# willake/cpu-ray-tracer

Measured on AMD Instinct MI355X. Metric: Mrays/sec (primary+secondary), 1280x720 64spp path trace — pipelined throughput over 878 consecutive 64-spp windows of one progressive render (single_render = one such render alone), higher is better.
Workload: dtype f32; 1 GPU; bunny_scene.xml FileScene BVH-SAH path tracer, 1280x720, 64 spp/step (passes=1, depthLimit=5); 1 step = 64 frames = the next spp window of a progressive render; the 878 steps are one crt_render job (14 render kernel launch(es), a wavefront per (tile, 128 consecutive frames), + ordered accumulate), one sync at the end; triangles=4968, parallelism=tile-wave x1

## Files before the change

cpu-ray-tracer_amd/__init__.py:

```python
import ctypes as C
import os
import subprocess

import numpy as np

HERE = os.path.dirname(os.path.abspath(__file__))
REPO = os.path.dirname(HERE)
LIB_PATH = os.environ.get("CRT_LIB_PATH") or os.path.join(HERE, "libcrt_amd.so")

SCENE_FILE, SCENE_TLAS = 0, 1
UPDATE_TRANSFORMS, UPDATE_BOUNDS = 1, 2
ACCEL_KDTREE, ACCEL_GRID = 1, 2
KD_NODE_DTYPE = np.dtype([("aabbMin", "<f4", 3), ("left", "<i4"), ("aabbMax", "<f4", 3), ("right", "<i4"), ("splitDistance", "<f4"), ("splitAxis", "<i4"),
                          ("firstTri", "<u4"), ("triCount", "<u4")])


class CrtError(RuntimeError):
    def __init__(self, code, msg):
        super().__init__("crt error %d: %s" % (code, msg))
        self.code = code


class Config(C.Structure):
    _fields_ = [("width", C.c_int32), ("height", C.c_int32), ("depthLimit", C.c_int32), ("device", C.c_int32),
# ... 516 lines not shown
        side = getattr(self, "_side_stream", None)
        if side is None:
            side = self._side_stream = torch.cuda.Stream(device=self.device)
        side.wait_stream(st)
        with torch.cuda.stream(side):
            out = run(side)
        st.wait_stream(side)
        for t in (out if isinstance(out, tuple) else (out,)):
            if isinstance(t, torch.Tensor):
                t.record_stream(st)
        return out

    def counters(self):
        c = CountersS()
        self._ck(self.L.crt_get_counters(self.h, C.byref(c)))
        return {n: int(getattr(c, n)) for n, _ in c._fields_}

    def reset_counters(self):
        self._ck(self.L.crt_reset_counters(self.h))

    def timing(self):
        t = TimingS()
        self._ck(self.L.crt_get_timing(self.h, C.byref(t)))
        return dict(render_kernel_ms=t.render_kernel_ms, resolve_kernel_ms=t.resolve_kernel_ms, render_launches=t.render_launches, pool_launches=t.pool_launches, split_launches=t.split_launches)

    def pool_lds(self, frames):
        self.L.crt_debug_pool_lds.restype = C.c_int
        self.L.crt_debug_pool_lds.argtypes = [C.c_void_p, C.c_uint32, C.c_void_p, C.c_void_p, C.c_void_p]
        b, lim, bits = C.c_uint32(), C.c_uint32(), C.c_uint32()
        if self.L.crt_debug_pool_lds(self.h, int(frames), C.byref(b), C.byref(lim), C.byref(bits)) != 0:
            raise CrtError(-3, "pool_lds: no scene uploaded")
        return b.value, lim.value, bits.value

    def tile_classes(self):
        self.L.crt_debug_tile_classes.restype = C.c_int
        self.L.crt_debug_tile_classes.argtypes = [C.c_void_p, C.c_void_p, C.c_uint32]
        n = self.L.crt_debug_tile_classes(self.h, None, 0)
        if n < 0:
            self._ck(n)
        out = np.zeros(n, np.uint8)
        if n:
            rc = self.L.crt_debug_tile_classes(self.h, _p(out), n)
            if rc < 0:
                self._ck(rc)
        return out

    def tile_clocks(self, tile_count):
        a = np.zeros((tile_count, 2), np.uint64)
        self._ck(self.L.crt_get_tile_clocks(self.h, _p(a)))
        return a

    def bind_accumulator(self, device_ptr):
        self._ck(self.L.crt_bind_accumulator(self.h, C.c_void_p(device_ptr)))

    def accumulator_device_ptr(self):
        p = C.c_void_p()
        self._ck(self.L.crt_accumulator_device_ptr(self.h, C.byref(p)))
        return p.value

def hit_fields(hits):
    import torch
    i = hits.view(torch.int32)
    return dict(t=hits[:, 0], u=hits[:, 1], v=hits[:, 2], objIdx=i[:, 3], triIdx=i[:, 4], traversed=i[:, 5], tested=i[:, 6])


def hit_info_fields(info):
    import torch
    return dict(I=info[:, 0:3], material=info.view(torch.int32)[:, 3], N=info[:, 4:7], u=info[:, 7], albedo=info[:, 8:11], v=info[:, 11])


class HostScene:

    def __init__(self, xml_path, kind, base_dir=None):
        self.L = lib()
        h = C.c_void_p()
# ... 325 lines not shown
def host_kd_build(positions):
    pos = np.ascontiguousarray(positions, np.float32).reshape(-1, 9)
    L = lib()
    info = (C.c_uint32 * 4)()

    def ck(rc):
        if rc != 0:
            raise CrtError(rc, L.crt_host_last_error().decode())
    ck(L.crt_host_kd_build(_p(pos), C.c_uint32(len(pos)), info, None, None))
    nodes = np.zeros(info[0], KD_NODE_DTYPE); r = np.zeros(max(info[1], 1), np.uint32)
    ck(L.crt_host_kd_build(_p(pos), C.c_uint32(len(pos)), None, _p(nodes), _p(r)))
    return dict(nodes=nodes, refs=r[:info[1]], maxDepth=int(info[2]), nodesUsed=int(info[3]))


def host_vertex_dedup(v8):
    v8 = np.ascontiguousarray(v8, np.float32).reshape(-1, 8)
    idx = np.zeros(len(v8), np.uint32); uniq = np.zeros((len(v8), 8), np.float32)
    L = lib(); L.crt_host_vertex_dedup.restype = C.c_uint32
    n = L.crt_host_vertex_dedup(v8.ctypes.data_as(C.c_void_p), C.c_uint32(len(v8)), idx.ctypes.data_as(C.c_void_p), uniq.ctypes.data_as(C.c_void_p))
    return idx, uniq[:n].copy()


def spp_window(rank, frames_per_rank, first_spp=1):
    return first_spp + rank * frames_per_rank


def tile_partition(rank, world, n_tiles):
    count = (n_tiles - rank + world - 1) // world if rank < n_tiles else 0
    return rank, world, count


TILE_NO_LIGHT, TILE_NO_FLOOR, TILE_NO_TREE = 1, 2, 4
TILE_SKY = 7


def tile_classes_host(camera, light_offsets, light_size, floor_d, root_pair, width, height, tile_first=0, tile_stride=1, tile_count=-1, flags=7):
    if tile_count < 0:
        tile_first, tile_stride, tile_count = 0, 1, (width // 16) * (height // 16)
    v = np.concatenate([np.asarray(camera, np.float32).reshape(12), np.asarray(light_offsets, np.float32).reshape(3), np.array([light_size, floor_d], np.float32),
                        np.asarray(root_pair, np.float32).reshape(16)]).astype(np.float32)
    out = np.zeros(tile_count, np.uint8)
    L = lib()
    L.crt_debug_tile_classes_host.restype = C.c_int
    L.crt_debug_tile_classes_host.argtypes = [C.c_void_p, C.c_uint32, C.c_int, C.c_int, C.c_uint32, C.c_uint32, C.c_uint32, C.c_void_p]
    rc = L.crt_debug_tile_classes_host(_p(v), flags, width, height, tile_first, tile_stride, tile_count, _p(out))
    if rc != 0:
        raise CrtError(rc, "crt_debug_tile_classes_host: invalid argument")
    return out


def reduce_accumulator(tensor, dist, dst=0):
    dist.reduce(tensor, dst=dst, op=dist.ReduceOp.SUM)
    return tensor


def allreduce_accumulator(tensor, dist):
    dist.all_reduce(tensor, op=dist.ReduceOp.SUM)
    return tensor
```

cpu-ray-tracer_amd/csrc/abi.cpp:

```cpp
#include "../../include/crt_abi.h"
#include "device/launch.h"
#include "device/tile_class.h"
#include "device/build_common.h"
#include "host/grid_resolution.h"

#include <cmath>
#include <cstdarg>
#include <cstddef>
#include <cstdio>
#include <cstdlib>
#include <cstring>
#include <deque>
#include <string>
#include <algorithm>
#include <vector>
#include <chrono>

static_assert(sizeof(crt_bvh_node) == 32 && sizeof(crt_tri) == 112 && sizeof(crt_tlas_node) == 32, "reference layouts");
static_assert(sizeof(crt::NodePair) == 64 && sizeof(crt::LeafTri) == 48 && sizeof(crt::ShadeTri) == 64 && sizeof(crt::TlasNode) == 32 &&
              sizeof(crt::Instance) == 128 && sizeof(crt::Material) == 32 && offsetof(crt::Instance, T) == 64, "device layouts");
static_assert(sizeof(crt_counters) == sizeof(crt::Counters), "counter layout");
static_assert(sizeof(crt_kd_node) == 48 && sizeof(crt::KdNode) == sizeof(crt_kd_node) && sizeof(crt::AltTri) == 48, "flat KD node (uploaded as it comes), alternative accelerators' triangle record");
static_assert(offsetof(crt::PrimDev, red) == 536 && sizeof(crt::PrimDev) == 552, "PrimDev: 134 floats, then the two texel pointers");
static_assert(sizeof(crt::BlasAltDesc) == 72, "BLAS descriptor");
// ... 957 lines not shown
    };
    float world[24];
    for (int i = 0; i < 8; i++) { world[3 * i] = (i & 1) ? c->meshHi[0] : c->meshLo[0]; world[3 * i + 1] = (i & 2) ? c->meshHi[1] : c->meshLo[1]; world[3 * i + 2] = (i & 4) ? c->meshHi[2] : c->meshLo[2]; }
    int wr[4] = {0, c->tilesX - 1, 0, c->tilesY - 1};
    (void)rect_of(world, wr);
    std::vector<uint32_t> first, second, rest;
    for (uint32_t i = 0; i < c->tileCount; i++) {
        const uint32_t tile = c->tileFirst + i * c->tileStride;
        const int tx = (int)(tile % (uint32_t)c->tilesX), ty = (int)(tile / (uint32_t)c->tilesX);
        const bool inRect = tx >= wr[0] && tx <= wr[1] && ty >= wr[2] && ty <= wr[3];
        if (inRect) first.push_back(i); else rest.push_back(i);
    }
    for (int k = 0; k <= crt_ctx::kLatStages; k++) { c->tuneCount[k] = 0; c->tuneMs[k] = 0; }
    c->latStage = 0; c->latBest = 0; c->latDone = false; c->latWarm = false; c->latConfirming = false; c->latQueue.clear(); c->costPending = false; c->latProbed = false;
    first.insert(first.end(), rest.begin(), rest.end());
    (void)sky_to_tail(c->hostClass, first);
    c->jobCostValid = false; c->jobCostPending = false; c->planValid = false; c->skyWindowTicks = 0;
    { const int r = upload_tile_order(c, first); if (r) return r; }
    c->orderDirty = false;
    return 0;
}

static int update_tile_class(crt_ctx* c)
{
    if (!c->classDirty || c->tileCount == 0) return 0;
    if (!c->dTileClass) HIPCK(c, hipMalloc((void**)&c->dTileClass, (size_t)c->tileCount));
    { const int r = order_behind_ahead(c); if (r) return r; }
    const int k = c->classFlip ^= 1;
    if (!c->hTileClass[k]) {
        HIPCK(c, hipHostMalloc((void**)&c->hTileClass[k], (size_t)c->tileCount, hipHostMallocDefault));
        HIPCK(c, ensure_event(&c->classCopied[k]));
    } else HIPCK(c, hipEventSynchronize(c->classCopied[k]));
    crt::classify_tiles(c->hScene, c->cfg.width, c->cfg.height, (uint32_t)c->tilesX, c->tileFirst, c->tileStride, c->tileCount, c->hTileClass[k]);
    {
        const uint8_t* cls = c->hTileClass[k];
        bool same = c->hostClass.size() == c->tileCount; uint32_t sky = 0;
        for (uint32_t i = 0; i < c->tileCount; i++) { const bool s = cls[i] == crt::kTileSky; sky += s ? 1u : 0u; if (same && s != (c->hostClass[i] == crt::kTileSky)) same = false; }
        c->hostClass.assign(cls, cls + c->tileCount); c->skyTiles = sky;
        if (!same) c->orderDirty = true;
    }
    HIPCK(c, hipMemcpyAsync(c->dTileClass, c->hTileClass[k], (size_t)c->tileCount, hipMemcpyHostToDevice, c->stream));
    HIPCK(c, hipEventRecord(c->classCopied[k], c->stream));
    c->orderReady = c->classCopied[k];
    c->classDirty = false;
    return 0;
}

static size_t sample_bytes_per_window(const crt_ctx* c, uint32_t passes) { return crt_slab_window_bytes(c->tileCount, passes); }
static size_t window_bytes(const crt_ctx* c, uint32_t passes) { return sample_bytes_per_window(c, passes) + (c->usePool ? crt_pool_scratch_bytes_per_window(c->tileCount) : 0); }

static uint32_t block_desc(uint32_t tile, uint32_t laneBase, uint32_t lanes, uint32_t window) { uint32_t lg = 0; while ((1u << lg) < lanes) lg++; return tile | (laneBase << 16) | (lg << 22) | (window << 25); }
static const uint32_t kLatLanes[7] = {64u, 32u, 16u, 8u, 4u, 2u, 1u};
static const double kLatG[7] = {1.0, 0.93, 0.88, 0.79, 0.69, 0.57, 0.48};
static int lat_index(uint32_t L) { int k = 0; while (k < 6 && kLatLanes[k] != L) k++; return k; }

static uint8_t next_lanes(uint8_t lanes, uint32_t cost, double T)
{
    int k = lat_index(lanes); const double unit = (double)cost / kLatG[k];
    while (k < 6 && unit * kLatG[k] > T) k++;
    while (k > 0 && unit * kLatG[k - 1] <= 0.9 * T) k--;
    return (uint8_t)kLatLanes[k];
}
extern "C" int crt_debug_next_lanes(const uint8_t* lanes, const uint32_t* cost, uint32_t n, double T, uint8_t* out)
{
    if (!lanes || !cost || !out) return CRT_ERR_INVALID;
    for (uint32_t i = 0; i < n; i++) { if (lanes[i] == 0 || lanes[i] > 64 || (64 % lanes[i]) != 0) return CRT_ERR_INVALID; out[i] = next_lanes(lanes[i], cost[i], T); }
// ... 2232 lines not shown
    if (e == hipSuccess) e = crt_launch_check_sqrt(d, c->stream);
    if (e == hipSuccess) e = hipMemcpyAsync(out, d, 16, hipMemcpyDeviceToHost, c->stream);
    if (e == hipSuccess) e = hipStreamSynchronize(c->stream);
    (void)hipFree(d);
    HIPCK(c, e);
    return CRT_OK;
}

extern "C" int crt_debug_primary_block(crt_ctx* c, float* out, float* camera, float* lightFloor)
{
    if (!c || !out) return CRT_ERR_INVALID;
    const crt::Scene& s = c->hScene;
    static_assert(offsetof(crt::Scene, primRoot) == offsetof(crt::Scene, rootPair) + 64 && offsetof(crt::Scene, primDown) + 12 == offsetof(crt::Scene, rootPair) + 64 + 4 * crt::kPrimFloats, "primary block");
    memcpy(out, s.rootPair, 64 + 4 * crt::kPrimFloats);
    if (camera) memcpy(camera, s.camPos, 48);
    if (lightFloor) { lightFloor[0] = s.lightInvT[7]; lightFloor[1] = s.lightInvT[3]; lightFloor[2] = s.lightInvT[11]; lightFloor[3] = s.floorD; }
    return CRT_OK;
}
extern "C" int crt_debug_primary_block_host(int op, const float* in, float* out)
{
    static crt::Scene s{};
    if (!in || !out || op < 0 || op > 2) return CRT_ERR_INVALID;
    if (op == 0) {
        s = crt::Scene{};
        s.camPos[2] = -2; s.topLeft[0] = -1; s.topLeft[1] = 1; s.topRight[0] = 1; s.topRight[1] = 1; s.bottomLeft[0] = -1; s.bottomLeft[1] = -1;
        memcpy(s.lightInvT, in, 48); s.floorD = in[12]; memcpy(s.rootPair, in + 13, 64); s.rootIsPair = 1;
    } else if (op == 1) { memcpy(s.camPos, in, 12); memcpy(s.topLeft, in + 3, 12); memcpy(s.topRight, in + 6, 12); memcpy(s.bottomLeft, in + 9, 12); }
    else memcpy(s.rootPair, in, 64);
    crt::set_primary(s);
    memcpy(out, s.rootPair, 64 + 4 * crt::kPrimFloats);
    return CRT_OK;
}

extern "C" int crt_debug_tile_classes(crt_ctx* c, uint8_t* out, uint32_t cap)
{
    if (!c || (!out && cap)) return CRT_ERR_INVALID;
    HIPCK(c, hipSetDevice(c->cfg.device));
    { const int r = update_tile_class(c); if (r) return r; }
    const uint32_t n = cap < c->tileCount ? cap : c->tileCount;
    if (n) {
        HIPCK(c, hipMemcpyAsync(out, c->dTileClass, n, hipMemcpyDeviceToHost, c->stream));
        HIPCK(c, hipStreamSynchronize(c->stream));
    }
    return (int)c->tileCount;
}
extern "C" int crt_debug_tile_classes_host(const float* in, uint32_t flags, int W, int H, uint32_t tileFirst, uint32_t tileStride, uint32_t tileCount, uint8_t* out)
{
    if (!in || !out || W < 16 || H < 16 || tileStride == 0) return CRT_ERR_INVALID;
    const uint32_t tilesX = (uint32_t)(W / 16), tiles = tilesX * (uint32_t)(H / 16);
    if (tileCount && (unsigned long long)tileFirst + (unsigned long long)(tileCount - 1) * tileStride >= tiles) return CRT_ERR_INVALID;
    crt::Scene s{};
    memcpy(s.camPos, in, 12); memcpy(s.topLeft, in + 3, 12); memcpy(s.topRight, in + 6, 12); memcpy(s.bottomLeft, in + 9, 12);
    s.W = W; s.H = H; s.invW = 1.0f / W; s.invH = 1.0f / H;
    s.lightInvT[0] = s.lightInvT[5] = s.lightInvT[10] = 1.0f; s.lightInvT[3] = in[12]; s.lightInvT[7] = in[13]; s.lightInvT[11] = in[14];
    s.lightSize = in[15]; s.floorN[1] = 1.0f; s.floorD = in[16];
    memcpy(s.rootPair, in + 17, 64);
    s.lightAxis = flags & 1u; s.floorAxisY = (flags >> 1) & 1u; s.rootIsPair = (flags >> 2) & 1u;
    crt::set_primary(s);
    crt::classify_tiles(s, W, H, tilesX, tileFirst, tileStride, tileCount, out);
    return CRT_OK;
}

static int device_probe(crt_ctx* c, int op, const void* in, void* out, uint32_t n)
{
    static const uint8_t words[18][2] = {{1, 1}, {1, 1}, {2, 1}, {1, 1}, {2, 1}, {6, 7}, {1, 18}, {4, 1}, {5, 3}, {13, 2}, {16, 4}, {2, 2}, {2, 2}, {2, 2}, {2, 2}, {4, 2}, {2, 1}, {5, 3}};
    if (!c || !in || !out || op < 0 || op > 17 || n > (1u << 25)) return CRT_ERR_INVALID;
    if (n == 0) return CRT_OK;
    const size_t inBytes = (size_t)n * words[op][0] * 4, outBytes = (size_t)n * words[op][1] * 4;
    HIPCK(c, hipSetDevice(c->cfg.device));
    char* d = nullptr;
    HIPCK(c, hipMalloc((void**)&d, inBytes + outBytes));
    hipError_t e = hipMemcpyAsync(d, in, inBytes, hipMemcpyHostToDevice, c->stream);
    if (e == hipSuccess) e = (op <= 10 || op == 17) ? crt_launch_probe_f32(op, d, d + inBytes, n, c->stream) : crt_launch_probe_f64(op, d, d + inBytes, n, c->stream);
    if (e == hipSuccess) e = hipMemcpyAsync(out, d + inBytes, outBytes, hipMemcpyDeviceToHost, c->stream);
    if (e == hipSuccess) e = hipStreamSynchronize(c->stream);
    (void)hipFree(d);
    HIPCK(c, e);
    return CRT_OK;
}
// ... 126 lines not shown
```

cpu-ray-tracer_amd/csrc/device/layout.h:

```cpp
#pragma once
#include <stdint.h>

namespace crt {

constexpr uint32_t kRefInterior = 0x80000000u;
constexpr uint32_t kRefTlasBit = 0x40000000u;
constexpr uint32_t kRefTlasInterior = 0x40000000u;
constexpr uint32_t kRefTlasLeaf = 0xC0000000u;
constexpr uint32_t kRefReturn = 0xFFFFFFFFu;
constexpr uint32_t kRefDone = 0u;
constexpr uint32_t kRefOffsetMask = 0x3fffffffu;
constexpr uint64_t kMaxGeomBytes = 1ull << 32;

constexpr uint32_t kRef16Interior = 0x8000u, kRef16TlasBit = 0x4000u, kRef16TlasLeaf = 0xC000u, kRef16TagMask = 0xC000u, kRef16IndexMask = 0x3fffu;
constexpr uint32_t kRef16Return = 0xFFFFu, kRef16MaxIndex = 0x3ffeu;
constexpr uint32_t kRefWideMaxIndex = 0x3ffffffeu;
struct PoolRefForm { uint32_t interior, tlasBit, tlasLeaf, tagMask, indexMask, ret; };
constexpr PoolRefForm pool_ref_form(uint32_t bits)
{
    return bits == 32u ? PoolRefForm{kRefInterior, kRefTlasBit, kRefTlasLeaf, 0xC0000000u, kRefOffsetMask, kRefReturn}
                       : PoolRefForm{kRef16Interior, kRef16TlasBit, kRef16TlasLeaf, kRef16TagMask, kRef16IndexMask, kRef16Return};
}

struct alignas(16) NodeChild { float lo[3]; uint32_t ref; float hi[3]; uint32_t ref16; };
// ... 46 lines not shown
    uint32_t tlasOff, instOff, shadeOff;
    uint32_t leafOff, tlasPairOff;
    uint32_t rootRef16, poolRefBits;
    const uint32_t* texels;
    const Material* mats;
    uint32_t rootRef;
    uint32_t stackDepth;
    uint32_t bvhStack;
    uint32_t lightAxis, floorAxisY;
    uint32_t rootIsPair;
    float rootPair[16];
    float primRoot[12];
    float primLight[3];
    float primFloor;
    float primRight[3], primDown[3];
};
constexpr uint32_t kPrimFloats = 22u;

inline void set_primary(Scene& s)
{
    const float* O = s.camPos;
    for (int c = 0; c < 2; c++)
        for (int k = 0; k < 3; k++) {
            s.primRoot[6 * c + k] = s.rootPair[8 * c + k] - O[k];
            s.primRoot[6 * c + 3 + k] = s.rootPair[8 * c + 4 + k] - O[k];
        }
    s.primLight[0] = O[1] + s.lightInvT[7]; s.primLight[1] = O[0] + s.lightInvT[3]; s.primLight[2] = O[2] + s.lightInvT[11];
    s.primFloor = O[1] + s.floorD;
    for (int k = 0; k < 3; k++) { s.primRight[k] = s.topRight[k] - s.topLeft[k]; s.primDown[k] = s.bottomLeft[k] - s.topLeft[k]; }
}

constexpr uint32_t kTileNoLight = 1u, kTileNoFloor = 2u, kTileNoTree = 4u;
constexpr uint32_t kTileSky = kTileNoLight | kTileNoFloor | kTileNoTree;

struct Counters { unsigned long long v[8]; };

struct alignas(16) RefitPlanRec { uint32_t pair, child[2], pad; };
constexpr uint32_t kPlanInterior = 0x80000000u;

struct alignas(64) TlasBuildHeader {
    uint32_t status;
    uint32_t step;
    uint32_t height;
    uint32_t searches;
    uint32_t staleA;
    uint32_t pad[11];
};
constexpr uint32_t kTlasBuildOk = 0u, kTlasBuildNoCandidate = 1u, kTlasBuildNoEnd = 2u;
constexpr uint32_t kTlasMaxBlas = 256u;

#if defined(__HIPCC__)
#define CRT_HOST_DEVICE __host__ __device__
#else
#define CRT_HOST_DEVICE
#endif
template <class TriCountOf>
CRT_HOST_DEVICE inline bool hit_record_ok(int32_t objIdx, int32_t triIdx, uint32_t objects, TriCountOf&& triCountOf)
{
    if (objIdx < 2) return objIdx >= -1;
    if ((uint32_t)(objIdx - 2) >= objects) return false;
    return triIdx >= 0 && (uint32_t)triIdx < triCountOf((uint32_t)(objIdx - 2));
}

struct KdNode { float lo[3]; int32_t left; float hi[3]; int32_t right; float splitDistance; int32_t splitAxis; uint32_t firstTri, triCount; };
struct AltTri { float v0[3]; uint32_t triIdx; float e1[3]; int32_t objIdx; float e2[3]; uint32_t pad; };
struct AltAccelDev {
// ... 57 lines not shown
```

cpu-ray-tracer_amd/csrc/device/render_pool.hip:

```cpp
#include <type_traits>
#include "launch.h"
#include "sample_body.h"

namespace crt {

enum : uint32_t {
    F_OX = 0, F_OY, F_OZ, F_DX, F_DY, F_DZ,
    F_RX, F_RY, F_RZ,
    F_T,
    F_SEED, F_META,
    F_U, F_V,
    F_COUNT,
    F_CUR = F_U, F_PEND = F_V,
    F_TRI = F_RX
};
constexpr uint32_t kMetaItemMask = 0x7ffu, kMetaDepthShift = 11u, kMetaInside = 1u << 14, kMetaFresh = 1u << 15, kMetaObjShift = 16u, kMetaLowMask = 0xffffu;
constexpr uint32_t kQueueMask = 127u;

#ifndef CRT_POOL_MIN_WAVES
#define CRT_POOL_MIN_WAVES 4
#endif
#ifndef CRT_POOL_WIDE_MIN_WAVES
#define CRT_POOL_WIDE_MIN_WAVES 4
#endif
// ... 45 lines not shown
__device__ __forceinline__ uint32_t rank_in(uint64_t m) { return __builtin_amdgcn_mbcnt_hi((uint32_t)(m >> 32), __builtin_amdgcn_mbcnt_lo((uint32_t)m, 0u)); }

template <int KIND, bool COUNT, int S, int REFBITS = 16>
__global__ __launch_bounds__(64, REFBITS == 32 ? CRT_POOL_WIDE_MIN_WAVES : CRT_POOL_MIN_WAVES) void render_pool_kernel(const Scene sc, char* __restrict__ slab, float* __restrict__ facScratch, Counters* __restrict__ counters,
                                                             unsigned long long* __restrict__ tileClocks, const uint32_t* __restrict__ tileOrder,
                                                             uint32_t tileFirst, uint32_t tileStride, uint32_t tileCount, uint32_t tilesX,
                                                             uint32_t sppFirst, uint32_t frames, uint32_t passes, uint32_t groups, uint32_t waveFrames, const uint32_t* __restrict__ waveTab, uint32_t tabBlocks, uint32_t longFrames,
                                                             uint32_t rankFirst, uint32_t* __restrict__ tileCost, unsigned long long* __restrict__ launchClk, const uint8_t* __restrict__ tileClass)
{
    extern __shared__ uint32_t lds[];
    const uint32_t lane = threadIdx.x;
#ifdef CRT_POOL_TIMELINE
    const unsigned long long tl0 = wall_clock64();
#endif
    const unsigned long long clk0 = (COUNT || tileCost) ? wall_clock64() : 0ull;
    if (launchClk && lane == 0) { atomicMax(&launchClk[0], ~clk0); atomicMax(&launchClk[1], clk0); }
    uint32_t rank0, grp, wf = waveFrames, first = 0u, limit = frames;
    if (waveTab) {
        if (blockIdx.x < tabBlocks) {
            uint32_t lo = 0u, hi = tileCount - rankFirst;
            while (hi - lo > 1u) { const uint32_t mid = (lo + hi) >> 1; if (waveTab[2u * mid] <= blockIdx.x) lo = mid; else hi = mid; }
            rank0 = lo; grp = blockIdx.x - waveTab[2u * lo]; wf = waveTab[2u * lo + 1u]; limit = longFrames;
        } else { const uint32_t b = blockIdx.x - tabBlocks; rank0 = b / groups; grp = b - rank0 * groups; wf = (uint32_t)S; first = longFrames; }
    } else { rank0 = blockIdx.x / groups; grp = blockIdx.x - rank0 * groups; }
    const uint32_t rank = rank0 + rankFirst;
    if (rank >= tileCount) return;
    const uint32_t tl = tileOrder ? tileOrder[rank] : rank;
    const uint32_t frame0 = first + grp * wf;
    if (frame0 >= limit) return;
    const uint32_t nOwn = (limit - frame0 < wf) ? limit - frame0 : wf;
    const uint32_t nStreams = nOwn < (uint32_t)S ? nOwn : (uint32_t)S;
    const uint32_t tile = tileFirst + tl * tileStride;
    const uint32_t tx = tile % tilesX, ty = tile / tilesX;
    const uint32_t tcls = tileClass ? __builtin_amdgcn_readfirstlane((uint32_t)tileClass[tl]) : 0u;
    auto not_sky = [&]() -> bool { return fresh(tcls) != kTileSky; };
    const char* __restrict__ geom = sc.geom;
    float* __restrict__ fac = facScratch + (size_t)blockIdx.x * (15u * (uint32_t)S);

    constexpr PoolRefForm R = pool_ref_form((uint32_t)REFBITS);
    using StackEntry = std::conditional_t<REFBITS == 32, uint32_t, uint16_t>;
    constexpr uint32_t kEntryB = (uint32_t)sizeof(StackEntry), kLevelB = 64u * kEntryB;
    char* const ldsB = reinterpret_cast<char*>(lds);
    const uint32_t laneB = lane * kEntryB;
    uint32_t* st = lds + (sc.stackDepth + 1u) * (kLevelB / 4u);
    float* stf = reinterpret_cast<float*>(st);
    uint8_t* qEnd = reinterpret_cast<uint8_t*>(st + F_COUNT * S);
    uint8_t* qBnc = qEnd + 128, * qRdy = qEnd + 256;
    uint16_t* slotFrame = reinterpret_cast<uint16_t*>(qEnd + 384);
    auto stk_top = [&](uint32_t at) -> uint32_t { return *reinterpret_cast<const StackEntry*>(ldsB + at); };
    auto stk_put = [&](uint32_t at, uint32_t v) { *reinterpret_cast<StackEntry*>(ldsB + at) = (StackEntry)v; };

    Cnt cn; cn.rays = cn.primary = cn.interior = cn.leaf = cn.tri = cn.tlas = cn.visits = cn.meshhits = 0;
    uint32_t trips = 0;
#ifdef CRT_POOL_DENS
    uint32_t dens[48]; for (int i = 0; i < 48; i++) dens[i] = 0;
    uint32_t live = nStreams; unsigned long long liveClk = wall_clock64();
#endif
    const uint32_t items = 256u * passes;
    const uint32_t rowLen = 64u * passes;
    const f3 nil3 = mk3(0.0f, 0.0f, 0.0f);

    for (uint32_t s = lane; s < nStreams; s += 64u) {
        st[F_SEED * S + s] = stream_seed(tx, ty, (uint32_t)sc.W, sppFirst, frame0 + s, passes);
        st[F_META * S + s] = kMetaFresh;
        qEnd[s] = (uint8_t)s;
        if (S > 64) slotFrame[s] = (uint16_t)s;
    }
// ... 35 lines not shown
                    if (allFinite) { d1 = box_fast_rel(ra0, ra1, rD, nh.t); d2 = box_fast_rel(rb0, rb1, rD, nh.t); }
                    else { d1 = box_exact_rel(ra0, ra1, rD, nh.t); d2 = box_exact_rel(rb0, rb1, rD, nh.t); }
                } else if (allFinite) { d1 = box_fast(a0, a1, O, rD, nh.t); d2 = box_fast(b0, b1, O, rD, nh.t); }
                else { d1 = box_exact(a0, a1, O, rD, nh.t); d2 = box_exact(b0, b1, O, rD, nh.t); }
                const Ordered o = ordered_step(d1, d2, asu(a1.w), asu(b1.w));
                pend = o.push ? o.farRef : 0u;
                ncur = o.hitN ? o.nearRef : kRefDone;
                if (COUNT) { if (KIND == 0) cn.interior++; else cn.tlas++; }
            } else ncur = sc.rootRef16;
            if (COUNT && KIND == 0 && (ncur & R.tagMask) == 0u && ncur != kRefDone) cn.leaf++;
            if (!PRIM || not_sky()) {
                stf[F_OX * S + s] = O.x; stf[F_OY * S + s] = O.y; stf[F_OZ * S + s] = O.z;
                stf[F_RX * S + s] = rD.x; stf[F_RY * S + s] = rD.y; stf[F_RZ * S + s] = rD.z;
                stf[F_T * S + s] = nh.t;
                st[F_CUR * S + s] = ncur; st[F_PEND * S + s] = pend;
            }
            stf[F_DX * S + s] = D.x; stf[F_DY * S + s] = D.y; stf[F_DZ * S + s] = D.z;
            st[F_SEED * S + s] = seed; st[F_META * S + s] = meta | ((uint32_t)(nh.objIdx + 1) << kMetaObjShift);
        }
        uint64_t mW = 0ull, mE = mAct, mB = 0ull;
        if (!PRIM || not_sky()) {
            const uint32_t depth = (meta >> kMetaDepthShift) & 7u;
            mW = mAct & mask_ne(ncur, kRefDone);
            const uint64_t mStop = mask_ule((uint32_t)(nh.objIdx + 1), 1u) | mask_sge((int)depth, sc.depthLimit);
            mE = mAct & ~mW & mStop; mB = mAct & ~mW & ~mStop;
            if (lane_in(mW)) qRdy[(rdyT + rank_in(mW)) & kQueueMask] = (uint8_t)s;
            if (lane_in(mB)) qBnc[(bncT + rank_in(mB)) & kQueueMask] = (uint8_t)s;
            rdyT += (uint32_t)__popcll(mW); bncT += (uint32_t)__popcll(mB);
        }
        CRT_DENS(20, __popcll(mAct)); CRT_DENS(19, __popcll(mW));
        if (lane_in(mE)) qEnd[(endT + rank_in(mE)) & kQueueMask] = (uint8_t)s;
        endT += (uint32_t)__popcll(mE);
    };
    auto world_ray = [&]() {
        tO = mk3(stf[F_OX * S + sid], stf[F_OY * S + sid], stf[F_OZ * S + sid]);
        tD = mk3(stf[F_DX * S + sid], stf[F_DY * S + sid], stf[F_DZ * S + sid]);
        trD = mk3(stf[F_RX * S + sid], stf[F_RY * S + sid], stf[F_RZ * S + sid]);
    };

    uint64_t mNode2 = 0ull;
    auto node_step = [&](auto exactTag, uint64_t m) {
        constexpr bool allFinite = !decltype(exactTag)::value;
        if (lane_in(m)) {
            if (COUNT) { if (KIND == 1 && (cur & R.tlasBit) != 0u) cn.tlas++; else cn.interior++; }
            const uint32_t top = stk_top(spB);
            float d1, d2;
            if constexpr (allFinite) { d1 = box_fast(q0, q1, tO, trD, h.t); d2 = box_fast(q2, q3, tO, trD, h.t); }
            else { d1 = box_exact(q0, q1, tO, trD, h.t); d2 = box_exact(q2, q3, tO, trD, h.t); }
            const Ordered o = ordered_step(d1, d2, asu(q1.w), asu(q3.w));
            stk_put(spB + kLevelB, o.farRef);
            const bool pop = !o.hitN && spB != laneB;
            cur = o.hitN ? o.nearRef : (pop ? top : kRefDone);
            spB = spB + (o.push ? kLevelB : 0u) - (pop ? kLevelB : 0u);
            if (COUNT && (cur & R.tagMask) == 0u && cur != kRefDone) cn.leaf++;
        }
    };
    auto record_offset = [&]() -> uint32_t {
        const uint32_t idx = cur & R.indexMask;
        const bool inter = (cur & R.interior) != 0u;
        uint32_t oa = idx * (inter ? 64u : 48u) + (inter ? 0u : sc.leafOff - 48u);
        if (KIND == 1 && (cur & R.tlasBit) != 0u)
            oa = (cur & R.interior) ? sc.instOff + idx * 128u : sc.tlasPairOff + idx * 64u;
        return oa;
    };
    auto load_records = [&](uint64_t m) {
        const uint32_t oa = record_offset();
// ... 73 lines not shown
                mBack = (mNode | mTriAll) & __builtin_amdgcn_ballot_w64(cur == R.ret);
                if (mBack != 0ull) {
                    if (lane_in(mBack)) {
                        world_ray();
                        const bool pop = spB != laneB;
                        const uint32_t top = stk_top(spB);
                        cur = pop ? top : kRefDone; spB -= pop ? kLevelB : 0u;
                        if (COUNT && (cur & R.tagMask) == 0u && cur != kRefDone) cn.leaf++;
                    }
                    mFinite = (mFinite & ~mBack) | (mBack & finite3_mask(trD));
                }
            }
            asm volatile("" ::: "memory");
            const uint64_t mFin = mRes & __builtin_amdgcn_ballot_w64(cur == kRefDone);
            if (mFin != 0ull) {
                CRT_DENS(5, 1); CRT_DENS(6, __popcll(mFin));
                const uint32_t depth = (metaLo >> kMetaDepthShift) & 7u;
                const uint64_t mStop = __builtin_amdgcn_ballot_w64((uint32_t)(h.objIdx + 1) <= 1u) | __builtin_amdgcn_ballot_w64((int)depth >= sc.depthLimit);
                const uint64_t mE = mFin & mStop, mB = mFin & ~mStop;
                if (lane_in(mFin)) {
                    stf[F_T * S + sid] = h.t; stf[F_U * S + sid] = h.u; stf[F_V * S + sid] = h.v;
                    st[F_TRI * S + sid] = (uint32_t)h.triIdx;
                    st[F_META * S + sid] = metaLo | ((uint32_t)(h.objIdx + 1) << kMetaObjShift);
                }
                if (lane_in(mE)) qEnd[(endT + rank_in(mE)) & kQueueMask] = (uint8_t)sid;
                if (lane_in(mB)) qBnc[(bncT + rank_in(mB)) & kQueueMask] = (uint8_t)sid;
                endT += (uint32_t)__popcll(mE); bncT += (uint32_t)__popcll(mB);
                mRes &= ~mFin;
            }
            asm volatile("" ::: "memory");
        }
        CRT_PSTAMP(p1); CRT_PACC(0, p0, p1);
        if (COUNT) trips++;
        CRT_DENS(0, 1);
#ifdef CRT_POOL_STAMPS
        pst[9]++;
#endif
#ifdef CRT_POOL_DENS
        dens[32u + CRT_LIVE_BUCKET(live)]++;
#endif
        {
            const uint32_t nRdy = rdyT - rdyH;
            const uint64_t mFree = ~mRes;
            if (nRdy != 0u) if (ctl_free(mRes)) {
                const uint32_t myRank = rank_in(mFree);
                const uint64_t mTake = mFree & __builtin_amdgcn_ballot_w64(myRank < nRdy);
                CRT_DENS(7, 1); CRT_DENS(8, __popcll(mTake));
                if (lane_in(mTake)) {
                    sid = qRdy[(rdyH + myRank) & kQueueMask];
                    tO = mk3(stf[F_OX * S + sid], stf[F_OY * S + sid], stf[F_OZ * S + sid]);
                    tD = mk3(stf[F_DX * S + sid], stf[F_DY * S + sid], stf[F_DZ * S + sid]);
                    trD = mk3(stf[F_RX * S + sid], stf[F_RY * S + sid], stf[F_RZ * S + sid]);
                    const uint32_t meta = st[F_META * S + sid];
                    h.t = stf[F_T * S + sid]; h.objIdx = (int)(meta >> kMetaObjShift) - 1; h.u = 0; h.v = 0; h.triIdx = -1;
                    metaLo = meta & kMetaLowMask;
                    cur = st[F_CUR * S + sid];
                    const uint32_t pend = st[F_PEND * S + sid];
                    stk_put(laneB + kLevelB, pend);
                    spB = laneB + (pend ? kLevelB : 0u);
                }
                mFinite = (mFinite & ~mTake) | (mTake & finite3_mask(trD));
                mRes |= mTake;
                rdyH += (uint32_t)__popcll(mTake);
            }
            if (mRes != 0ull) {
                CRT_DENS(21, 1);
                uint32_t oa = record_offset();
                if (!lane_in(mRes)) oa = 0u;
                q0 = ldp<0>(geom, oa); q1 = ldp<1>(geom, oa); q2 = ldp<2>(geom, oa); q3 = ldp<3>(geom, oa);
            }
        }
        asm volatile("" ::: "memory");
        const uint32_t nEnd = endT - endH, nBnc = bncT - bncH;
        uint32_t walking = pop32(mRes) + (rdyT - rdyH), fullest = nEnd | nBnc;
        asm("" : "+s"(walking));
        walking = fullest >= 64u ? 0u : walking;
        asm("" : "+s"(walking), "+s"(fullest));
        if (walking < (uint32_t)CRT_POOL_STARVE) {
            const uint32_t run = fullest >= 64u ? (nEnd >> 6) | ((nBnc >> 6) << 8) : (nEnd >= nBnc ? nEnd : nBnc << 8);
            const uint32_t runEnd = run & 0xffu, runBnc = run >> 8;

            CRT_PSTAMP(p2b); CRT_PACC(1, p1, p2b);
            if (runEnd != 0u) {
                const uint32_t n = nEnd < 64u ? nEnd : 64u;
                const uint64_t mActE = mask_ult(lane, n);
                const bool act = lane_in(mActE);
                const uint32_t s = act ? qEnd[(endH + lane) & kQueueMask] : 0u;
                endH += n;
                uint32_t meta = 0, seed = 0; int obj = -1; f3 D = nil3;
                if (act) { meta = st[F_META * S + s]; seed = st[F_SEED * S + s]; obj = (int)(meta >> kMetaObjShift) - 1; D = mk3(stf[F_DX * S + s], stf[F_DY * S + s], stf[F_DZ * S + s]); }
                const int depth = (int)((meta >> kMetaDepthShift) & 7u);
                uint32_t item = meta & kMetaItemMask;
                const uint64_t mFirst = mask_ne(meta & kMetaFresh, 0u), mEnded = mActE & ~mFirst, mMiss = mEnded & mask_eq(meta >> kMetaObjShift, 0u);
                const bool first = lane_in(mFirst), ended = lane_in(mEnded), miss = lane_in(mMiss);
#ifdef CRT_POOL_DENS
                dens[36u + CRT_LIVE_BUCKET(live)]++;
#endif
                CRT_DENS(9, 1); CRT_DENS(10, n); CRT_DENS_MASK(11, miss); CRT_DENS_MASK(13, act && first); CRT_DENS_MASK(25, ended && depth > 0); CRT_DENS_MASK(26, ended && depth > 1); CRT_DENS_MASK(27, ended && depth > 2);
                if (ended && obj >= 2) cn.meshhits++;
                float fk[15];
#pragma unroll
                for (int k = 0; k < 5; k++) {
                    fk[3 * k] = fk[3 * k + 1] = fk[3 * k + 2] = 0.0f;
                    if (not_sky()) if (ended && depth > k) {
#pragma unroll
                        for (int j = 0; j < 3; j++) fk[3 * k + j] = __hip_atomic_load(fac + (3 * k + j) * S + s, __ATOMIC_RELAXED, __HIP_MEMORY_SCOPE_AGENT);
                    }
                }
                uint32_t skyTexel = 0u;
                if (miss) {
                    float phi, theta; sky_angles(D, phi, theta);
                    const kernarg_f sk = scene_floats(offsetof(Scene, skyOffset));
                    skyTexel = sc.texels[tex_index(asu(sk[0]), (int)asu(sk[1]), (int)asu(sk[2]), phi * CRT_INV2PI, theta * CRT_INVPI)];
                }
                bool gen = act && first;
                size_t sampleAt = 0;
                if (ended) {
                    uint32_t pix = item, pass = 0;
                    if (fresh(passes) != 1u) { pix = item / passes; pass = item - pix * passes; }
                    const uint32_t fr = frame0 + (S > 64 ? (uint32_t)slotFrame[s] : s);
                    sampleAt = slab_position(fr, tileCount, tl, pix, rowLen, passes, pass);
                    item++;
                    gen = item < items;
                }
                uint64_t mGen = mFirst | (mEnded & mask_ult(item, items));
                const uint64_t mDone = mEnded & ~mGen;
                if (mDone != 0ull) {
                    uint64_t mTake = 0ull;
                    if (S > 64) if (nextFrame < nOwn) {
                        const uint32_t f = nextFrame + rank_in(mDone);
                        mTake = mDone & mask_ult(f, nOwn);
                        if (lane_in(mTake)) {
                            slotFrame[s] = (uint16_t)f;
                            seed = stream_seed(tx, ty, (uint32_t)sc.W, sppFirst, frame0 + f, passes);
                            item = 0u;
                        }
                        nextFrame += pop32(mTake);
                        mGen |= mTake;
                    }
                    nLive -= pop32(mDone & ~mTake);
                }
                gen = lane_in(mGen);
#ifdef CRT_POOL_DENS
                {
                    const uint32_t gone = (uint32_t)__popcll(__builtin_amdgcn_ballot_w64(ended) & ~__builtin_amdgcn_ballot_w64(gen));
                    if (gone) { const unsigned long long now = wall_clock64(); dens[44u + CRT_LIVE_BUCKET(live)] += (uint32_t)(now - liveClk); liveClk = now; live -= gone; }
                }
#endif
                const kernarg_f cam = scene_floats(offsetof(Scene, camPos));
                const f3 camPos = mk3(cam[0], cam[1], cam[2]);
                f3 v = camPos;
                if (gen) {
                    const uint32_t pix = (fresh(passes) == 1u) ? item : item / passes;
                    const f3 TL = mk3(cam[3], cam[4], cam[5]);
                    constexpr size_t pc = (offsetof(Scene, primRight) - offsetof(Scene, camPos)) / 4;
                    const f3 right = mk3(cam[pc], cam[pc + 1], cam[pc + 2]), down = mk3(cam[pc + 3], cam[pc + 4], cam[pc + 5]);
                    v = primary_target(camPos, TL, right, down, cam[12], cam[13], tx, ty, pix, seed);
                    cn.primary++;
                }
                CRT_DENS_MASK(12, gen);
                CRT_PSTAMP(e1); CRT_PACC(2, p2b, e1);
                new_ray(std::true_type{}, mGen, s, v, true, camPos, seed, item);
                CRT_PSTAMP(e2); CRT_PACC(3, e1, e2);
                if (ended) {
                    f3 L = miss ? tex_unpack(skyTexel) : ((depth >= sc.depthLimit) ? mk3(0, 0, 0) : mk3(24, 24, 22));
                    if (not_sky()) {
#pragma unroll
                        for (int k = 4; k >= 0; k--)
                            if (depth > k) L = mk3(fk[3 * k], fk[3 * k + 1], fk[3 * k + 2]) * L;
                    }
                    store_sample(slab, sampleAt, L);
                }
#ifdef CRT_POOL_STAMPS
                { CRT_PSTAMP(e3); CRT_PACC(4, e2, e3); pst[10]++; }
#endif
                asm volatile("" :: "v"(fk[0]), "v"(fk[1]), "v"(fk[2]), "v"(fk[3]), "v"(fk[4]), "v"(fk[5]), "v"(fk[6]), "v"(fk[7]), "v"(fk[8]), "v"(fk[9]), "v"(fk[10]), "v"(fk[11]), "v"(fk[12]), "v"(fk[13]), "v"(fk[14]), "v"(skyTexel));
            }
            CRT_PSTAMP(p3);
            asm volatile("" ::: "memory");
            if (runBnc != 0u) {
                const uint32_t n = nBnc < 64u ? nBnc : 64u;
                const uint64_t mActB = mask_ult(lane, n);
                const bool act = lane_in(mActB);
                const uint32_t s = act ? qBnc[(bncH + lane) & kQueueMask] : 0u;
                bncH += n;
                f3 O = nil3, D = nil3; float ht = 0, hu = 0, hv = 0; int obj = 1; uint32_t tri = 0, seed = 0, meta = 0;
                if (act) {
                    tri = st[F_TRI * S + s];
                    O = mk3(stf[F_OX * S + s], stf[F_OY * S + s], stf[F_OZ * S + s]);
                    D = mk3(stf[F_DX * S + s], stf[F_DY * S + s], stf[F_DZ * S + s]);
                    ht = stf[F_T * S + s]; hu = stf[F_U * S + s]; hv = stf[F_V * S + s];
                    seed = st[F_SEED * S + s]; meta = st[F_META * S + s]; obj = (int)(meta >> kMetaObjShift) - 1;
                }
                const bool mesh = act && obj >= 2;
#ifdef CRT_POOL_DENS
                dens[40u + CRT_LIVE_BUCKET(live)]++;
#endif
                CRT_DENS(14, 1); CRT_DENS(15, n); CRT_DENS_MASK(16, mesh);
                rec4 s0 = {0, 0, 0, 0}, s1 = s0, s2 = s0, s3 = s0;
                if (mesh) { const uint32_t so = sc.shadeOff + tri * 64u; s0 = ldp<0>(geom, so); s1 = ldp<1>(geom, so); s2 = ldp<2>(geom, so); s3 = ldp<3>(geom, so); cn.meshhits++; }
                const bool inside = (meta & kMetaInside) != 0u;
                const int depth = (int)((meta >> kMetaDepthShift) & 7u);
                const uint32_t item = meta & kMetaItemMask;
                f3 v = O; bool newInside = false;
                if (act) {
                    const f3 I = O + ht * D;
                    SurfPoint p;
                    if (obj == 1) {
                        const kernarg_f fl = scene_floats(offsetof(Scene, floorN));
                        const kernarg_f fm = scene_floats(offsetof(Scene, floorMat));
                        const rec4 m0 = {fm[0], fm[1], fm[2], fm[3]}, m1 = {fm[4], fm[5], fm[6], fm[7]};
                        p = floor_point(mk3(fl[0], fl[1], fl[2]), fl[4], m0, m1, I);
                    } else p = mesh_point<KIND>(s0, s1, s2, s3, hu, hv, obj, geom, sc.instOff, sc.mats);
                    const f3 N = face_ray(p.N, D);
                    uint32_t texel = 0x00ffffffu;
                    if (p.tW > 0) texel = sc.texels[tex_index(p.tOff, p.tW, p.tH, p.tu, p.tv)];
                    const f3 medium = medium_of(inside, p.absorb, ht);
                    CRT_PSTAMP(b1); CRT_PACC(5, p3, b1);
                    const Bounce b = draw_bounce(seed, D, N, inside, p.refl, p.refr);
                    newInside = b.newInside;
                    const f3 c = (p.tW > 0) ? tex_unpack(texel) : mk3(1.0f, 1.0f, 1.0f);
                    CRT_PSTAMP(b2); CRT_PACC(6, b1, b2);
                    const float inv = rcp_exact(sqrt_exact(dot3(b.v, b.v)));
                    const f3 nv = b.branch == kDiffuse ? b.v * inv : b.v;
                    v = nv;
                    const f3 factor = bounce_factor(b.branch, c, medium, nv, N);
                    float* fd = fac + (3 * depth) * S + s;
                    __hip_atomic_store(fd, factor.x, __ATOMIC_RELAXED, __HIP_MEMORY_SCOPE_AGENT);
                    __hip_atomic_store(fd + S, factor.y, __ATOMIC_RELAXED, __HIP_MEMORY_SCOPE_AGENT);
                    __hip_atomic_store(fd + 2 * S, factor.z, __ATOMIC_RELAXED, __HIP_MEMORY_SCOPE_AGENT);
                    O = I + nv * CRT_EPS;
// ... 117 lines not shown
```

cpu-ray-tracer_amd/csrc/device/tile_class.h:

```cpp
#pragma once
#include <cmath>
#include <cstring>
#include "layout.h"

namespace crt {

inline void classify_tiles(const Scene& s, int W, int H, uint32_t tilesX, uint32_t tileFirst, uint32_t tileStride, uint32_t tileCount, uint8_t* cls)
{
    if (tileCount == 0) return;
    memset(cls, 0, tileCount);
    if (W <= 0 || H <= 0 || tilesX == 0) return;
    const double cam[3] = {s.camPos[0], s.camPos[1], s.camPos[2]};
    double TL[3], R[3], Dn[3];
    for (int k = 0; k < 3; k++) { TL[k] = s.topLeft[k]; R[k] = (double)s.topRight[k] - s.topLeft[k]; Dn[k] = (double)s.bottomLeft[k] - s.topLeft[k]; }
    const bool wantTree = s.rootIsPair != 0, wantFloor = s.floorAxisY != 0, wantLight = s.lightAxis != 0;
    if (!wantTree && !wantFloor && !wantLight) return;

    double mag = 0; bool finite = true;
    auto see = [&](double x) { if (!std::isfinite(x)) finite = false; else if (std::fabs(x) > mag) mag = std::fabs(x); };
    for (int k = 0; k < 3; k++) { see(cam[k]); see(TL[k]); see(s.topRight[k]); see(s.bottomLeft[k]); see(TL[k] + R[k] + Dn[k]); }
    if (wantTree) for (int c = 0; c < 2; c++) for (int k = 0; k < 3; k++) { see(s.rootPair[8 * c + k]); see(s.rootPair[8 * c + 4 + k]); }
    if (wantLight) { see(s.lightInvT[3]); see(s.lightInvT[7]); see(s.lightInvT[11]); see(s.lightSize); see(s.primLight[0]); see(s.primLight[1]); see(s.primLight[2]); }
    if (wantFloor) { see(s.floorD); see(s.primFloor); }
    see(s.invW); see(s.invH);
    const double rr = R[0] * R[0] + R[1] * R[1] + R[2] * R[2], dd = Dn[0] * Dn[0] + Dn[1] * Dn[1] + Dn[2] * Dn[2], rd = R[0] * Dn[0] + R[1] * Dn[1] + R[2] * Dn[2];
    if (!finite || !(rr > 0) || !(dd > 0)) return;
    const double invW = s.invW, invH = s.invH;
    const double step = std::fmin(std::sqrt(rr) * std::fabs(invW), std::sqrt(dd) * std::fabs(invH));
    if (!(step >= std::ldexp(mag, -16)) || !(invW > 0) || !(invH > 0)) return;
    const double tau = std::ldexp(mag, -18);

    auto ray = [&](double px, double py, double v[3]) { for (int k = 0; k < 3; k++) v[k] = TL[k] + (px * invW) * R[k] + (py * invH) * Dn[k] - cam[k]; };

    bool tree = wantTree; double bx0 = 1e300, bx1 = -1e300, by0 = 1e300, by1 = -1e300;
    if (tree) {
        const double N[3] = {R[1] * Dn[2] - R[2] * Dn[1], R[2] * Dn[0] - R[0] * Dn[2], R[0] * Dn[1] - R[1] * Dn[0]};
        const double num = (TL[0] - cam[0]) * N[0] + (TL[1] - cam[1]) * N[1] + (TL[2] - cam[2]) * N[2];
        const double det = rr * dd - rd * rd;
        if (!(det > 1e-12 * rr * dd) || num == 0) tree = false;
        for (int c = 0; c < 2 && tree; c++)
            for (int i = 0; i < 8 && tree; i++) {
                double d[3];
                for (int k = 0; k < 3; k++) d[k] = (double)s.rootPair[8 * c + ((i >> k) & 1 ? 4 : 0) + k] - cam[k];
                const double den = d[0] * N[0] + d[1] * N[1] + d[2] * N[2];
                const double t = den != 0 ? num / den : -1;
                if (!(t > 0) || !(t <= 16)) { tree = false; break; }
                double Q[3]; for (int k = 0; k < 3; k++) Q[k] = cam[k] + t * d[k] - TL[k];
                const double qr = Q[0] * R[0] + Q[1] * R[1] + Q[2] * R[2], qd = Q[0] * Dn[0] + Q[1] * Dn[1] + Q[2] * Dn[2];
                const double px = (qr * dd - qd * rd) / det / invW, py = (qd * rr - qr * rd) / det / invH;
                if (!std::isfinite(px) || !std::isfinite(py)) { tree = false; break; }
                bx0 = std::fmin(bx0, px); bx1 = std::fmax(bx1, px); by0 = std::fmin(by0, py); by1 = std::fmax(by1, py);
            }
    }

    const double fnum = s.primFloor;
    const bool floorOk = wantFloor && fnum != 0;
    const double lOy = s.primLight[0], lOx = s.primLight[1], lOz = s.primLight[2], lsize = s.lightSize;
    const bool lightOk = wantLight && lOy != 0;

    for (uint32_t i = 0; i < tileCount; i++) {
        const uint32_t tile = tileFirst + i * tileStride;
        const double x0 = 16.0 * (tile % tilesX) - 1.0, x1 = x0 + 18.0, y0 = 16.0 * (tile / tilesX) - 1.0, y1 = y0 + 18.0;
        double v[4][3];
        ray(x0, y0, v[0]); ray(x1, y0, v[1]); ray(x0, y1, v[2]); ray(x1, y1, v[3]);
        double vyMin = v[0][1], vyMax = v[0][1];
        for (int j = 1; j < 4; j++) { vyMin = std::fmin(vyMin, v[j][1]); vyMax = std::fmax(vyMax, v[j][1]); }
        const bool up = vyMin >= tau, down = vyMax <= -tau;
        uint8_t b = 0;
        if (tree && (x1 < bx0 || x0 > bx1 || y1 < by0 || y0 > by1)) b |= kTileNoTree;
        if (floorOk && (fnum > 0 ? up : down)) b |= kTileNoFloor;
        if (lightOk) {
            double q[4], qMax = 0, vMax = 0;
            for (int j = 0; j < 4; j++) { q[j] = -v[j][1] / lOy; qMax = std::fmax(qMax, std::fabs(q[j])); vMax = std::fmax(vMax, std::fmax(std::fabs(v[j][0]), std::fabs(v[j][2]))); }
            const double m = std::ldexp(qMax * (std::fabs(lOx) + std::fabs(lOz) + std::fabs(lsize)) + vMax, -16), qTau = tau / std::fabs(lOy);
            bool behind = true, xHi = true, xLo = true, zHi = true, zLo = true;
            for (int j = 0; j < 4; j++) {
                behind = behind && q[j] <= -qTau;
                xHi = xHi && v[j][0] - (lsize - lOx) * q[j] >= m; xLo = xLo && v[j][0] + (lsize + lOx) * q[j] <= -m;
                zHi = zHi && v[j][2] - (lsize - lOz) * q[j] >= m; zLo = zLo && v[j][2] + (lsize + lOz) * q[j] <= -m;
            }
            if (std::isfinite(m) && (behind || xHi || xLo || zHi || zLo)) b |= kTileNoLight;
        }
        cls[i] = b;
    }
}

}
```

Baseline: 34410 Mrays/s.

## Add floor-only tile class and resolve primary rays analytically against floor plane

Extends host tile classification with a FLOOR_SURE bit set when every camera ray in a tile points toward the floor plane. Tiles that also miss the light and the BVH root are marked as floor tiles. The pool kernel then computes the primary-ray hit distance in closed form and enqueues the ray straight into the bounce queue, skipping BVH traversal. The debug APIs mask the new bit for compatibility. This adds a conservative geometric test, and the per-tile branch is wave-uniform because the class is read with readfirstlane.

```diff
diff --git a/cpu-ray-tracer_amd/__init__.py b/cpu-ray-tracer_amd/__init__.py
--- a/cpu-ray-tracer_amd/__init__.py
+++ b/cpu-ray-tracer_amd/__init__.py
@@ -572,15 +572,16 @@
             raise CrtError(-3, "pool_lds: no scene uploaded")
         return b.value, lim.value, bits.value
 
-    def tile_classes(self):
-        self.L.crt_debug_tile_classes.restype = C.c_int
-        self.L.crt_debug_tile_classes.argtypes = [C.c_void_p, C.c_void_p, C.c_uint32]
-        n = self.L.crt_debug_tile_classes(self.h, None, 0)
+    def tile_classes(self, ex=False):
+        f = self.L.crt_debug_tile_classes_ex if ex else self.L.crt_debug_tile_classes
+        f.restype = C.c_int
+        f.argtypes = [C.c_void_p, C.c_void_p, C.c_uint32]
+        n = f(self.h, None, 0)
         if n < 0:
             self._ck(n)
         out = np.zeros(n, np.uint8)
         if n:
-            rc = self.L.crt_debug_tile_classes(self.h, _p(out), n)
+            rc = f(self.h, _p(out), n)
             if rc < 0:
                 self._ck(rc)
         return out
@@ -972,18 +973,21 @@
 
 TILE_NO_LIGHT, TILE_NO_FLOOR, TILE_NO_TREE = 1, 2, 4
 TILE_SKY = 7
-
-
-def tile_classes_host(camera, light_offsets, light_size, floor_d, root_pair, width, height, tile_first=0, tile_stride=1, tile_count=-1, flags=7):
+TILE_FLOOR_SURE = 8
+TILE_FLOOR = TILE_NO_LIGHT | TILE_NO_TREE | TILE_FLOOR_SURE
+
+
+def tile_classes_host(camera, light_offsets, light_size, floor_d, root_pair, width, height, tile_first=0, tile_stride=1, tile_count=-1, flags=7, ex=False):
     if tile_count < 0:
         tile_first, tile_stride, tile_count = 0, 1, (width // 16) * (height // 16)
     v = np.concatenate([np.asarray(camera, np.float32).reshape(12), np.asarray(light_offsets, np.float32).reshape(3), np.array([light_size, floor_d], np.float32),
                         np.asarray(root_pair, np.float32).reshape(16)]).astype(np.float32)
     out = np.zeros(tile_count, np.uint8)
     L = lib()
-    L.crt_debug_tile_classes_host.restype = C.c_int
-    L.crt_debug_tile_classes_host.argtypes = [C.c_void_p, C.c_uint32, C.c_int, C.c_int, C.c_uint32, C.c_uint32, C.c_uint32, C.c_void_p]
-    rc = L.crt_debug_tile_classes_host(_p(v), flags, width, height, tile_first, tile_stride, tile_count, _p(out))
+    f = L.crt_debug_tile_classes_host_ex if ex else L.crt_debug_tile_classes_host
+    f.restype = C.c_int
+    f.argtypes = [C.c_void_p, C.c_uint32, C.c_int, C.c_int, C.c_uint32, C.c_uint32, C.c_uint32, C.c_void_p]
+    rc = f(_p(v), flags, width, height, tile_first, tile_stride, tile_count, _p(out))
     if rc != 0:
         raise CrtError(rc, "crt_debug_tile_classes_host: invalid argument")
     return out
diff --git a/cpu-ray-tracer_amd/csrc/abi.cpp b/cpu-ray-tracer_amd/csrc/abi.cpp
--- a/cpu-ray-tracer_amd/csrc/abi.cpp
+++ b/cpu-ray-tracer_amd/csrc/abi.cpp
@@ -1013,6 +1013,8 @@
         HIPCK(c, ensure_event(&c->classCopied[k]));
     } else HIPCK(c, hipEventSynchronize(c->classCopied[k]));
     crt::classify_tiles(c->hScene, c->cfg.width, c->cfg.height, (uint32_t)c->tilesX, c->tileFirst, c->tileStride, c->tileCount, c->hTileClass[k]);
+    if (hook("CRT_DEBUG_NO_FLOOR_CLASS"))
+        for (uint32_t i = 0; i < c->tileCount; i++) c->hTileClass[k][i] &= (uint8_t)~crt::kTileFloorSure;
     {
         const uint8_t* cls = c->hTileClass[k];
         bool same = c->hostClass.size() == c->tileCount; uint32_t sky = 0;
@@ -3311,7 +3313,7 @@
     return CRT_OK;
 }
 
-extern "C" int crt_debug_tile_classes(crt_ctx* c, uint8_t* out, uint32_t cap)
+extern "C" int crt_debug_tile_classes_ex(crt_ctx* c, uint8_t* out, uint32_t cap)
 {
     if (!c || (!out && cap)) return CRT_ERR_INVALID;
     HIPCK(c, hipSetDevice(c->cfg.device));
@@ -3323,7 +3325,20 @@
     }
     return (int)c->tileCount;
 }
+extern "C" int crt_debug_tile_classes(crt_ctx* c, uint8_t* out, uint32_t cap)
+{
+    const int r = crt_debug_tile_classes_ex(c, out, cap);
+    for (uint32_t i = 0; r > 0 && i < cap && i < (uint32_t)r; i++) out[i] &= (uint8_t)crt::kTileNoMask;
+    return r;
+}
+extern "C" int crt_debug_tile_classes_host_ex(const float* in, uint32_t flags, int W, int H, uint32_t tileFirst, uint32_t tileStride, uint32_t tileCount, uint8_t* out);
 extern "C" int crt_debug_tile_classes_host(const float* in, uint32_t flags, int W, int H, uint32_t tileFirst, uint32_t tileStride, uint32_t tileCount, uint8_t* out)
+{
+    const int r = crt_debug_tile_classes_host_ex(in, flags, W, H, tileFirst, tileStride, tileCount, out);
+    for (uint32_t i = 0; r == CRT_OK && i < tileCount; i++) out[i] &= (uint8_t)crt::kTileNoMask;
+    return r;
+}
+extern "C" int crt_debug_tile_classes_host_ex(const float* in, uint32_t flags, int W, int H, uint32_t tileFirst, uint32_t tileStride, uint32_t tileCount, uint8_t* out)
 {
     if (!in || !out || W < 16 || H < 16 || tileStride == 0) return CRT_ERR_INVALID;
     const uint32_t tilesX = (uint32_t)(W / 16), tiles = tilesX * (uint32_t)(H / 16);
diff --git a/cpu-ray-tracer_amd/csrc/device/layout.h b/cpu-ray-tracer_amd/csrc/device/layout.h
--- a/cpu-ray-tracer_amd/csrc/device/layout.h
+++ b/cpu-ray-tracer_amd/csrc/device/layout.h
@@ -102,6 +102,9 @@
 
 constexpr uint32_t kTileNoLight = 1u, kTileNoFloor = 2u, kTileNoTree = 4u;
 constexpr uint32_t kTileSky = kTileNoLight | kTileNoFloor | kTileNoTree;
+constexpr uint32_t kTileFloorSure = 8u;
+constexpr uint32_t kTileFloor = kTileNoLight | kTileNoTree | kTileFloorSure;
+constexpr uint32_t kTileNoMask = 7u;
 
 struct Counters { unsigned long long v[8]; };
 
diff --git a/cpu-ray-tracer_amd/csrc/device/render_pool.hip b/cpu-ray-tracer_amd/csrc/device/render_pool.hip
--- a/cpu-ray-tracer_amd/csrc/device/render_pool.hip
+++ b/cpu-ray-tracer_amd/csrc/device/render_pool.hip
@@ -101,7 +101,7 @@
     const uint32_t nStreams = nOwn < (uint32_t)S ? nOwn : (uint32_t)S;
     const uint32_t tile = tileFirst + tl * tileStride;
     const uint32_t tx = tile % tilesX, ty = tile / tilesX;
-    const uint32_t tcls = tileClass ? __builtin_amdgcn_readfirstlane((uint32_t)tileClass[tl]) : 0u;
+    const uint32_t tcls = tileClass ? __builtin_amdgcn_readfirstlane((uint32_t)tileClass[tl] & (sc.depthLimit > 0 ? ~0u : ~kTileFloorSure)) : 0u;
     auto not_sky = [&]() -> bool { return fresh(tcls) != kTileSky; };
     const char* __restrict__ geom = sc.geom;
     float* __restrict__ fac = facScratch + (size_t)blockIdx.x * (15u * (uint32_t)S);
@@ -203,6 +203,23 @@
         if (lane_in(mE)) qEnd[(endT + rank_in(mE)) & kQueueMask] = (uint8_t)s;
         endT += (uint32_t)__popcll(mE);
     };
+    auto floor_ray = [&](uint64_t mAct, uint32_t s, f3 v, f3 O, uint32_t seed, uint32_t meta) {
+        if (lane_in(mAct)) {
+            const float inv = rcp_exact(sqrt_exact(dot3(v, v)));
+            const f3 D = v * inv;
+            cn.rays++;
+            if (COUNT) { if (KIND == 0) cn.interior++; else cn.tlas++; }
+            const kernarg_f pf = scene_floats(offsetof(Scene, primFloor));
+            const float t = -pf[0] / D.y;
+            stf[F_OX * S + s] = O.x; stf[F_OY * S + s] = O.y; stf[F_OZ * S + s] = O.z;
+            stf[F_DX * S + s] = D.x; stf[F_DY * S + s] = D.y; stf[F_DZ * S + s] = D.z;
+            stf[F_T * S + s] = t;
+            st[F_SEED * S + s] = seed; st[F_META * S + s] = meta | (2u << kMetaObjShift);
+            qBnc[(bncT + rank_in(mAct)) & kQueueMask] = (uint8_t)s;
+        }
+        CRT_DENS(20, __popcll(mAct));
+        bncT += (uint32_t)__popcll(mAct);
+    };
     auto world_ray = [&]() {
         tO = mk3(stf[F_OX * S + sid], stf[F_OY * S + sid], stf[F_OZ * S + sid]);
         tD = mk3(stf[F_DX * S + sid], stf[F_DY * S + sid], stf[F_DZ * S + sid]);
@@ -342,7 +359,7 @@
         }
         CRT_PSTAMP(p1); CRT_PACC(0, p0, p1);
         if (COUNT) trips++;
-        CRT_DENS(0, 1);
+        CRT_DENS(0, 1); CRT_DENS(30, tcls == kTileFloor);
 #ifdef CRT_POOL_STAMPS
         pst[9]++;
 #endif
@@ -406,7 +423,7 @@
 #ifdef CRT_POOL_DENS
                 dens[36u + CRT_LIVE_BUCKET(live)]++;
 #endif
-                CRT_DENS(9, 1); CRT_DENS(10, n); CRT_DENS_MASK(11, miss); CRT_DENS_MASK(13, act && first); CRT_DENS_MASK(25, ended && depth > 0); CRT_DENS_MASK(26, ended && depth > 1); CRT_DENS_MASK(27, ended && depth > 2);
+                CRT_DENS(9, 1); CRT_DENS(31, tcls == kTileFloor); CRT_DENS(10, n); CRT_DENS_MASK(11, miss); CRT_DENS_MASK(13, act && first); CRT_DENS_MASK(25, ended && depth > 0); CRT_DENS_MASK(26, ended && depth > 1); CRT_DENS_MASK(27, ended && depth > 2);
                 if (ended && obj >= 2) cn.meshhits++;
                 float fk[15];
 #pragma unroll
@@ -470,7 +487,8 @@
                 }
                 CRT_DENS_MASK(12, gen);
                 CRT_PSTAMP(e1); CRT_PACC(2, p2b, e1);
-                new_ray(std::true_type{}, mGen, s, v, true, camPos, seed, item);
+                if (fresh(tcls) != kTileFloor) new_ray(std::true_type{}, mGen, s, v, true, camPos, seed, item);
+                if (fresh(tcls) == kTileFloor) floor_ray(mGen, s, v, camPos, seed, item);
                 CRT_PSTAMP(e2); CRT_PACC(3, e1, e2);
                 if (ended) {
                     f3 L = miss ? tex_unpack(skyTexel) : ((depth >= sc.depthLimit) ? mk3(0, 0, 0) : mk3(24, 24, 22));
@@ -506,7 +524,7 @@
 #ifdef CRT_POOL_DENS
                 dens[40u + CRT_LIVE_BUCKET(live)]++;
 #endif
-                CRT_DENS(14, 1); CRT_DENS(15, n); CRT_DENS_MASK(16, mesh);
+                CRT_DENS(14, 1); CRT_DENS(31, tcls == kTileFloor); CRT_DENS(15, n); CRT_DENS_MASK(16, mesh);
                 rec4 s0 = {0, 0, 0, 0}, s1 = s0, s2 = s0, s3 = s0;
                 if (mesh) { const uint32_t so = sc.shadeOff + tri * 64u; s0 = ldp<0>(geom, so); s1 = ldp<1>(geom, so); s2 = ldp<2>(geom, so); s3 = ldp<3>(geom, so); cn.meshhits++; }
                 const bool inside = (meta & kMetaInside) != 0u;
diff --git a/cpu-ray-tracer_amd/csrc/device/tile_class.h b/cpu-ray-tracer_amd/csrc/device/tile_class.h
--- a/cpu-ray-tracer_amd/csrc/device/tile_class.h
+++ b/cpu-ray-tracer_amd/csrc/device/tile_class.h
@@ -55,6 +55,7 @@
 
     const double fnum = s.primFloor;
     const bool floorOk = wantFloor && fnum != 0;
+    const bool sureOk = floorOk && std::fabs(fnum) < std::ldexp(1.0, 60) && std::fabs(fnum) >= std::ldexp(1.0, -60);
     const double lOy = s.primLight[0], lOx = s.primLight[1], lOz = s.primLight[2], lsize = s.lightSize;
     const bool lightOk = wantLight && lOy != 0;
 
@@ -69,6 +70,12 @@
         uint8_t b = 0;
         if (tree && (x1 < bx0 || x0 > bx1 || y1 < by0 || y0 > by1)) b |= kTileNoTree;
         if (floorOk && (fnum > 0 ? up : down)) b |= kTileNoFloor;
+        if (sureOk && (fnum > 0 ? down : up)) {
+            double vv = 0;
+            for (int j = 0; j < 4; j++) vv = std::fmax(vv, v[j][0] * v[j][0] + v[j][1] * v[j][1] + v[j][2] * v[j][2]);
+            const double vyAbsMin = fnum > 0 ? -vyMax : vyMin;
+            if (std::isfinite(vv) && vyAbsMin >= std::ldexp(std::sqrt(vv), -18)) b |= kTileFloorSure;
+        }
         if (lightOk) {
             double q[4], qMax = 0, vMax = 0;
             for (int j = 0; j < 4; j++) { q[j] = -v[j][1] / lOy; qMax = std::fmax(qMax, std::fabs(q[j])); vMax = std::fmax(vMax, std::fmax(std::fabs(v[j][0]), std::fabs(v[j][2]))); }
```

Result: faster. 34890 Mrays/s, median of 6 (+1.4%).
